# vinits5/learning3d

Measured on AMD Instinct MI355X. Metric: clouds/sec DGCNN-fwd+Chamfer B=32 N=1024; kNN HBM GB/s vs peak at 1/2/4/8 GPU, higher is better.
Workload: dtype f32 (shared-MLP GEMMs as f16x2: fp32 operands carried as an fp16 high part + an fp16 residual (unscaled between the EdgeConv kernel and conv5, 2^12-scaled elsewhere), 3 fp16 MFMA products per fp32 product, f32 accumulate, fp32-level error -- tests bound it by 2x the fp32-MFMA kernel's own error agai

## Files before the change

learning3d_amd/csrc/conv_f16.hip:

```cpp
#include <type_traits>
#include "common.h"
#include "split_bf16.h"
#include "split_f16.h"

typedef _Float16 f16x8 __attribute__((ext_vector_type(8)));

#define CF_TM 256
#define CF_TN 256
#define CF_WBYTES (6 * 4096)
#define CF_XBYTES (4 * 4096)
#define CF_STAGE (CF_WBYTES + CF_XBYTES)
#define CF_NSTAGE 3
#define CF_LDS (CF_NSTAGE * CF_STAGE)

typedef __attribute__((address_space(3))) void *cf_lds_ptr_t;
typedef const __attribute__((address_space(1))) void *cf_gbl_ptr_t;

__global__ __launch_bounds__(256) void cf_absmax_kernel(const float *__restrict__ src, size_t n, unsigned *__restrict__ out)
{
    float m = 0.f;
    const size_t gid = (size_t)blockIdx.x * 256 + threadIdx.x, gsz = (size_t)gridDim.x * 256;
    const size_t head = min(n, (size_t)((16 - ((size_t)src & 15)) & 15) / 4);
    const float4 *v = (const float4 *)(src + head);
    const size_t n4 = (n - head) / 4;
    size_t i = gid;
    for (; i + 3 * gsz < n4; i += 4 * gsz) {
        const float4 a = v[i], b = v[i + gsz], c = v[i + 2 * gsz], d = v[i + 3 * gsz];
        m = fmaxf(m, fmaxf(fmaxf(fmaxf(fabsf(a.x), fabsf(a.y)), fmaxf(fabsf(a.z), fabsf(a.w))),
                           fmaxf(fmaxf(fabsf(b.x), fabsf(b.y)), fmaxf(fabsf(b.z), fabsf(b.w)))));
        m = fmaxf(m, fmaxf(fmaxf(fmaxf(fabsf(c.x), fabsf(c.y)), fmaxf(fabsf(c.z), fabsf(c.w))),
                           fmaxf(fmaxf(fabsf(d.x), fabsf(d.y)), fmaxf(fabsf(d.z), fabsf(d.w)))));
    }
    for (; i < n4; i += gsz) {
        const float4 a = v[i];
        m = fmaxf(m, fmaxf(fmaxf(fabsf(a.x), fabsf(a.y)), fmaxf(fabsf(a.z), fabsf(a.w))));
    }
    for (size_t e = gid; e < head; e += gsz) m = fmaxf(m, fabsf(src[e]));
    for (size_t e = head + 4 * n4 + gid; e < n; e += gsz) m = fmaxf(m, fabsf(src[e]));
    for (int off = 32; off > 0; off >>= 1) m = fmaxf(m, __shfl_xor(m, off, 64));
    __shared__ float red[4];
    if ((threadIdx.x & 63) == 0) red[threadIdx.x >> 6] = m;
    __syncthreads();
    if (threadIdx.x == 0) {
        m = fmaxf(fmaxf(red[0], red[1]), fmaxf(red[2], red[3]));
        const unsigned bits = __float_as_uint(m);
        if (bits > __atomic_load_n(out, __ATOMIC_RELAXED)) atomicMax(out, bits);
    }
}

__global__ __launch_bounds__(256) void cf_absmax_rows_kernel(const float *__restrict__ src, long R, int C, long stride, unsigned *__restrict__ out)
{
    float m = 0.f;
    const long r0 = (long)blockIdx.x * 64, r1 = min(R, r0 + 64);
    for (long r = r0; r < r1; r++)
        for (int c = threadIdx.x; c < C; c += 256) m = fmaxf(m, fabsf(src[r * stride + c]));
    for (int off = 32; off > 0; off >>= 1) m = fmaxf(m, __shfl_xor(m, off, 64));
    if ((threadIdx.x & 63) == 0) atomicMax(out, __float_as_uint(m));
}

__device__ __forceinline__ int cf_clamp_exp(int s) { return s < -126 ? -126 : (s > 126 ? 126 : s); }

__device__ __forceinline__ int cf_scale_exp(float wmax)
{
    if (!(wmax > 0.f) || !(wmax < INFINITY)) return 0;
    int e;
    frexpf(wmax, &e);
    return cf_clamp_exp(3 - e);
}

__global__ __launch_bounds__(256) void cf_split_w_kernel(const float *__restrict__ src, int R, int C, const float *__restrict__ rinv,
                                                         uint4 *__restrict__ pH, uint4 *__restrict__ pHs, uint4 *__restrict__ pM)
{
    const int noct = (C + 7) / 8;
    const long id = (long)blockIdx.x * 256 + threadIdx.x;
    if (id >= (long)R * noct) return;
    const int row = (int)(id % R), o = (int)(id / R);
    const float up = 1.0f / rinv[row];
    _Float16 H[8], Hs[8], M[8];
#pragma unroll
    for (int e = 0; e < 8; e++) {
        const int k = o * 8 + e;
        const float v = (k < C ? src[(size_t)row * C + k] : 0.f) * up;
        H[e] = (_Float16)v;
        M[e] = (_Float16)(v - (float)H[e]);
        Hs[e] = (_Float16)((float)H[e] * 0x1p-12f);
    }
    pH[(size_t)o * R + row] = *(const uint4 *)H;
    pHs[(size_t)o * R + row] = *(const uint4 *)Hs;
    pM[(size_t)o * R + row] = *(const uint4 *)M;
}

__global__ __launch_bounds__(256) void cf_rowsum_kernel(const float *__restrict__ src, int R, int C, unsigned *__restrict__ out,
                                                        float *__restrict__ rinv)
{
    const int lane = threadIdx.x & 63, row = blockIdx.x * 4 + (threadIdx.x >> 6);
    float s = 0.f, mx = 0.f;
    if (row < R)
        for (int c = lane; c < C; c += 64) {
            const float a = fabsf(src[(size_t)row * C + c]);
            s += a;
            mx = fmaxf(mx, a);
        }
#pragma unroll
    for (int d = 32; d > 0; d >>= 1) {
        s += __shfl_xor(s, d, 64);
        mx = fmaxf(mx, __shfl_xor(mx, d, 64));
    }
    if (lane == 0 && row < R) rinv[row] = ldexpf(1.0f, -cf_scale_exp(mx));
    __shared__ float ws[4];
    if (lane == 0) ws[threadIdx.x >> 6] = s;
    __syncthreads();
    if (threadIdx.x == 0) atomicMax(out, __float_as_uint(fmaxf(fmaxf(ws[0], ws[1]), fmaxf(ws[2], ws[3]))));
}

__device__ __forceinline__ int cf_act_exp(float xmax)
{
    if (!(xmax > 0.f) || !(xmax < INFINITY)) return 0;
    int e;
    frexpf(xmax, &e);
    return cf_clamp_exp(12 - e);
}

__global__ __launch_bounds__(256) void cf_rowinv_act_kernel(const float *__restrict__ src, long R, int C, long stride, float *__restrict__ rinv)
{
    const int lane = threadIdx.x & 63;
    const long row = (long)blockIdx.x * 4 + (threadIdx.x >> 6);
    if (row >= R) return;
    float mx = 0.f;
    for (int c = lane; c < C; c += 64) mx = fmaxf(mx, fabsf(src[row * stride + c]));
#pragma unroll
    for (int d = 32; d > 0; d >>= 1) mx = fmaxf(mx, __shfl_xor(mx, d, 64));
    if (lane == 0) rinv[row] = ldexpf(1.0f, -cf_act_exp(mx));
}

template <bool CFIRST>
__global__ __launch_bounds__(256) void cf_split_x_kernel(const float *__restrict__ src, long R, int C, int Npts, const unsigned *__restrict__ amax,
                                                         uint4 *__restrict__ ph, uint4 *__restrict__ pm, float *__restrict__ inv,
                                                         int *__restrict__ range_flag)
{
    const int T = cf_act_exp(__uint_as_float(*amax));
    const float up = ldexpf(1.0f, T);
    if (blockIdx.x == 0 && threadIdx.x == 0) *inv = ldexpf(1.0f, -T);
    const int noct = (C + 7) / 8;
    const long id = (long)blockIdx.x * 256 + threadIdx.x;
    if (id >= R * noct) return;
    const long row = id % R;
    const int o = (int)(id / R);
    _Float16 h[8], m[8];
    float big = 0.f;
#pragma unroll
    for (int e = 0; e < 8; e++) {
        const int k = o * 8 + e;
        float v = 0.f;
        if (k < C) v = (CFIRST ? src[((size_t)(row / Npts) * C + k) * Npts + row % Npts] : src[(size_t)row * C + k]) * up;
        big = fmaxf(big, fabsf(v));
        h[e] = (_Float16)v;
        m[e] = (_Float16)((v - (float)h[e]) * 4096.0f);
    }
    ph[(size_t)o * R + row] = *(const uint4 *)h;
    pm[(size_t)o * R + row] = *(const uint4 *)m;
    if (!(big <= 60000.f) && range_flag) *(volatile int *)range_flag = 1;
}

#define CFS_ROWS 64
#define CFS_OCT 32
#define CFS_STRIDE (CFS_ROWS + 1)
__global__ __launch_bounds__(256) void cf_split_x_cl_kernel(const float *__restrict__ src, long R, int C, const unsigned *__restrict__ amax,
                                                            uint4 *__restrict__ ph, uint4 *__restrict__ pm, float *__restrict__ inv,
                                                            int *__restrict__ range_flag, long sstride = 0, float rs = 4096.0f,
                                                            const float *__restrict__ rinv = nullptr)
{
    if (sstride == 0) sstride = C;
    __shared__ uint4 lh[CFS_OCT * CFS_STRIDE], lm[CFS_OCT * CFS_STRIDE];
    const int T = cf_act_exp(__uint_as_float(*amax));
    const float up = ldexpf(1.0f, T);
    if (blockIdx.x == 0 && blockIdx.y == 0 && threadIdx.x == 0 && !rinv) *inv = ldexpf(1.0f, -T);
    const int t = threadIdx.x;
    const long row0 = (long)blockIdx.x * CFS_ROWS;
    const int o0 = blockIdx.y * CFS_OCT;
    float big = 0.f;
    {
        const int oc = t & 31, o = o0 + oc;
#pragma unroll
        for (int pass = 0; pass < CFS_ROWS / 8; pass++) {
            const int r = pass * 8 + (t >> 5);
            const long row = row0 + r;
            float v[8];
#pragma unroll
            for (int e = 0; e < 8; e++) v[e] = 0.f;
            float upr = up;
            if (row < R && o * 8 < C) {
                if (rinv) upr = 1.0f / rinv[row];
                const float *p = src + (size_t)row * sstride + o * 8;
                if (o * 8 + 8 <= C && (C & 3) == 0 && (sstride & 3) == 0 && (((size_t)src) & 15) == 0) {
                    const f32x4 a = *(const f32x4 *)p, b = *(const f32x4 *)(p + 4);
                    v[0] = a[0]; v[1] = a[1]; v[2] = a[2]; v[3] = a[3]; v[4] = b[0]; v[5] = b[1]; v[6] = b[2]; v[7] = b[3];
                } else {
#pragma unroll
                    for (int e = 0; e < 8; e++) if (o * 8 + e < C) v[e] = p[e];
                }
            }
            _Float16 h[8], m[8];
#pragma unroll
            for (int e = 0; e < 8; e++) {
                const float x = v[e] * upr;
                big = fmaxf(big, fabsf(x));
                h[e] = (_Float16)x;
                m[e] = (_Float16)((x - (float)h[e]) * rs);
            }
            lh[oc * CFS_STRIDE + r] = *(const uint4 *)h;
            lm[oc * CFS_STRIDE + r] = *(const uint4 *)m;
        }
    }
    __syncthreads();
    {
        const int r = t & 63;
        const long row = row0 + r;
        const int noct = (C + 7) / 8;
#pragma unroll
        for (int pass = 0; pass < CFS_OCT / 4; pass++) {
            const int oc = pass * 4 + (t >> 6), o = o0 + oc;
            if (row < R && o < noct) {
                ph[(size_t)o * R + row] = lh[oc * CFS_STRIDE + r];
                pm[(size_t)o * R + row] = lm[oc * CFS_STRIDE + r];
            }
        }
    }
    if (!(big <= 60000.f) && range_flag) *(volatile int *)range_flag = 1;
}

#ifdef CF_TIMELINE
__device__ long long *g_cf_timeline;
#define CFM(i) { if (threadIdx.x == 0) g_cf_timeline[(size_t)blockIdx.x * 8 + (i)] = __builtin_amdgcn_s_memrealtime(); }
#else
#define CFM(i)
#endif
template <bool NARROW, bool AMAX, bool GROUP, int NPW = 3, bool RESID = false, bool OUT2 = false, bool SHIFTN = false>
__global__ __launch_bounds__(512) void conv_f16_kernel(const uint4 *__restrict__ xh, const uint4 *__restrict__ xm,
                                                       const uint4 *__restrict__ wH, const uint4 *__restrict__ wHs,
                                                       const uint4 *__restrict__ wM, const float *__restrict__ winv,
                                                       const float *__restrict__ xinv, const float *__restrict__ scale, const float *__restrict__ shift,
                                                       int shift_bstride, int Bn, int Cin, int Cout, int N, int relu,
                                                       float *__restrict__ y, uint2 *__restrict__ oph, uint2 *__restrict__ opm,
                                                       float *__restrict__ oinv, const float *__restrict__ obs, float *__restrict__ ypool,
                                                       int pool, unsigned *__restrict__ amax_out, int amax_cdiv)
{
    constexpr int TM = NARROW ? 128 : CF_TM, TN = NARROW ? 512 : CF_TN;
    constexpr int WR = TM * 16, XR = TN * 16;
    static_assert(NPW == 3 || (NPW == 2 && !NARROW && !GROUP), "two weight planes: wide tile");
    static_assert(!RESID || (!NARROW && !AMAX && !GROUP), "residual epilogue: wide tile, fp32 output");
    static_assert(!OUT2 || (NPW == 2 && !AMAX && !RESID), "unscaled output image: the two-plane form");
    static_assert(!SHIFTN || (NPW == 2 && !AMAX && !RESID && !OUT2), "column-indexed shift: the plain two-plane form");
    constexpr int WBYTES = 2 * NPW * WR, STAGE = WBYTES + 4 * XR;
    constexpr int NPIECE = NARROW ? 6 : (NPW == 3 ? 5 : 4);
    extern __shared__ __attribute__((aligned(16))) unsigned char lds[];
    const int t = threadIdx.x, lane = t & 63, wave = t >> 6;
    const int wm = NARROW ? (wave & 1) : (wave & 3), wn = NARROW ? (wave >> 1) : (wave >> 2);
    CFM(0)
#ifdef CF_TIMELINE
    if (t == 0) { unsigned id; asm volatile("s_getreg_b32 %0, hwreg(HW_REG_HW_ID)" : "=s"(id)); g_cf_timeline[(size_t)blockIdx.x * 8 + 7] = id; }
#endif
    int pt, ct;
    {
        const int nct = Cout / TM, npt = Bn * (N / TN), L = blockIdx.x;
        if (npt % 8 == 0) {
            const int xcd = L & 7, slot = L >> 3;
            ct = slot % nct;
            pt = (slot / nct) * 8 + xcd;
        } else {
            ct = L % nct;
            pt = L / nct;
        }
    }
    const int ntn = N / TN;
    const int n0 = (pt % ntn) * TN, co0 = ct * TM, b = pt / ntn;
    const int nk = Cin / 16;
    const size_t BN = (size_t)Bn * N;

    const uint4 *src[NPIECE];
    size_t stride[NPIECE];
    int dst[NPIECE];
    constexpr int WQ = TM / 64, XQ = TN / 64, NWP = 2 * NPW * WQ, NXP = 4 * XQ;
#pragma unroll
    for (int i = 0; i < NPIECE; i++) {
        int q = wave * NPIECE + i;
        if (q >= NWP + NXP) q -= NXP;
        if (q < NWP) {
            const int reg = q / WQ, p = reg >> 1, kg = reg & 1, quarter = q % WQ;
            const uint4 *pl = p == 0 ? wH : ((NPW == 3 && p == 1) ? wHs : wM);
            src[i] = pl + (size_t)kg * Cout + co0 + quarter * 64 + lane;
            stride[i] = 2 * (size_t)Cout;
            dst[i] = reg * WR + quarter * 1024;
        } else {
            const int q2 = q - NWP, reg = q2 / XQ, p = reg >> 1, kg = reg & 1, quarter = q2 % XQ;
            const uint4 *pl = p == 0 ? xh : xm;
            src[i] = pl + (size_t)kg * BN + (size_t)b * N + n0 + quarter * 64 + lane;
            stride[i] = 2 * BN;
            dst[i] = WBYTES + reg * XR + quarter * 1024;
        }
    }
    auto issue_one = [&](int stage, int i) {
        __builtin_amdgcn_global_load_lds((cf_gbl_ptr_t)src[i], (cf_lds_ptr_t)(lds + stage * STAGE + dst[i]), 16, 0, 0);
        src[i] += stride[i];
    };
    auto issue = [&](int stage) {
#pragma unroll
        for (int i = 0; i < NPIECE; i++) issue_one(stage, i);
    };

    f32x16 acc[2][4];
#pragma unroll
    for (int a = 0; a < 2; a++)
#pragma unroll
        for (int c = 0; c < 4; c++)
#pragma unroll
            for (int r = 0; r < 16; r++) acc[a][c][r] = 0.f;

    const int kgl = lane >> 5;
    const int a_off = kgl * WR + (wm * 64 + (lane & 31)) * 16;
    const int b_off = WBYTES + kgl * XR + (wn * 128 + (lane & 31)) * 16;

    issue(0);
    if (nk > 1) issue(1);
    int stage = 0;
#ifdef CF_TIMING
    long long tq[5] = {0, 0, 0, 0, 0}, tp = __builtin_amdgcn_s_memtime();
#define CFT(n) { const long long now_ = __builtin_amdgcn_s_memtime(); tq[n] += now_ - tp; tp = now_; }
#else
#define CFT(n)
#endif
    for (int kc = 0; kc < nk; kc++) {
        CFT(4)
        if (kc + 1 >= nk) asm volatile("s_waitcnt vmcnt(0)" ::: "memory");
        else if (NARROW) asm volatile("s_waitcnt vmcnt(6)" ::: "memory");
        else if (NPW == 3) asm volatile("s_waitcnt vmcnt(5)" ::: "memory");
        else asm volatile("s_waitcnt vmcnt(4)" ::: "memory");
        CFT(0)
        __builtin_amdgcn_s_barrier();
#ifdef CF_TIMELINE
        if (kc == 0) CFM(1)
#endif
        CFT(1)
        const int nst = stage == 0 ? 2 : stage - 1;
        const bool more = kc + 2 < nk;
        CFT(2)
        const unsigned char *base = lds + stage * STAGE;
        f16x8 A[2][NPW], Bf[4][2];
#pragma unroll
        for (int p = 0; p < 2; p++)
#pragma unroll
            for (int c = 0; c < 4; c++) Bf[c][p] = *(const f16x8 *)(base + b_off + c * 512 + p * 2 * XR);
#pragma unroll
        for (int p = NPW - 1; p >= 0; p--)
#pragma unroll
            for (int a = 0; a < 2; a++) A[a][p] = *(const f16x8 *)(base + a_off + a * 512 + p * 2 * WR);
#pragma unroll
        for (int n = 0; n < 24; n++) {
            const int prod = n >> 3, a = (n >> 2) & 1, c = n & 3;
            const int pa = NPW == 3 ? (prod == 0 ? 2 : (prod == 1 ? 1 : 0)) : (prod == 0 ? 1 : 0);
            const int pb = prod == 1 ? 1 : 0;
            acc[a][c] = __builtin_amdgcn_mfma_f32_32x32x16_f16(A[a][pa], Bf[c][pb], acc[a][c], 0, 0, 0);
            constexpr int GAP = NARROW ? 4 : (NPW == 3 ? 5 : 6);
            if (n % GAP == 3) {
                __builtin_amdgcn_sched_barrier(0);
                if (more) issue_one(nst, n / GAP);
                __builtin_amdgcn_sched_barrier(0);
            }
        }
        stage = stage == 2 ? 0 : stage + 1;
        CFT(3)
    }
#ifdef CF_TIMING
    if (lane == 0) {
        long long *o = (long long *)y + ((size_t)blockIdx.x * 8 + wave) * 8;
        for (int n = 0; n < 5; n++) o[n] = tq[n];
    }
    {
        float keep = 0.f;
        for (int a = 0; a < 2; a++) for (int c = 0; c < 4; c++) for (int r = 0; r < 16; r++) keep += acc[a][c][r];
        if (keep == 12345.678f) y[0] = keep;
    }
    return;
#endif

    CFM(2)
    const float xinv0 = *xinv;
    const float *rinv = winv + 4;
    if (oph || ypool) {
        float up = 1.f;
        if (oph) {
            float bound = fmaf(obs[1] * winv[2], 4096.0f * *xinv, obs[0]) * 1.000001f;
            int e = 0;
            if (bound > 0.f && bound < 3.0e38f) (void)frexpf(bound, &e);
            const int To = cf_clamp_exp(12 - e);
            up = ldexpf(1.f, To);
            if (blockIdx.x == 0 && t == 0) *oinv = ldexpf(1.f, -To);
        }
      if constexpr (!GROUP) {
        const size_t rows = (size_t)Bn * N;
        const int half = lane >> 5, NP = N / 128;
#pragma unroll
        for (int a = 0; a < 2; a++)
#pragma unroll
            for (int gq = 0; gq < 4; gq++) {
                const int cob = co0 + wm * 64 + a * 32 + 8 * gq + 4 * half;
                float sc[4], sh[4], vmax[4];
#pragma unroll
                for (int u = 0; u < 4; u++) {
                    sc[u] = (scale ? scale[cob + u] : 1.f) * rinv[cob + u];
                    sh[u] = shift ? shift[(size_t)b * shift_bstride + cob + u] : 0.f;
                    vmax[u] = -INFINITY;
                }
#pragma unroll
                for (int c = 0; c < 4; c++) {
                    float v[4];
#pragma unroll
                    for (int u = 0; u < 4; u++) {
                        v[u] = acc[a][c][4 * gq + u] * sc[u] * xinv0 + sh[u];
                        if (relu) v[u] = l3d_act(v[u], relu);
                        vmax[u] = fmaxf(vmax[u], v[u]);
                    }
                    if (oph) {
                        uint32_t h0, h1, m0, m1;
                        if constexpr (OUT2) {
                            af_split_x_unscaled(v[0], v[1], up, h0, m0);
                            af_split_x_unscaled(v[2], v[3], up, h1, m1);
                        } else {
                            af_split_x(v[0], v[1], up, h0, m0);
                            af_split_x(v[2], v[3], up, h1, m1);
                        }
                        const size_t row = (size_t)b * N + n0 + wn * 128 + c * 32 + (lane & 31);
                        const size_t cellh = ((size_t)(cob >> 3) * rows + row) * 2 + half;
                        oph[cellh] = make_uint2(h0, h1);
                        opm[cellh] = make_uint2(m0, m1);
                    }
                }
                if (ypool) {
#pragma unroll
                    for (int u = 0; u < 4; u++) {
#pragma unroll
                        for (int d = 1; d < 32; d <<= 1) vmax[u] = fmaxf(vmax[u], __shfl_xor(vmax[u], d, 64));
                    }
                    if ((lane & 31) == 0) {
#pragma unroll
                        for (int u = 0; u < 4; u++)
                            ypool[((size_t)b * Cout + cob + u) * NP + (n0 + wn * 128) / 128] = vmax[u];
                    }
                }
            }
      } else {
        const size_t rows = (size_t)Bn * N;
        const int half = lane >> 5, NP = N / pool;
        const int span = pool < 32 ? pool : 32;
#pragma clang loop unroll(full)
        for (int a = 0; a < 2; a++)
#pragma clang loop unroll(full)
            for (int gq = 0; gq < 4; gq++) {
                const int cob = co0 + wm * 64 + a * 32 + 8 * gq + 4 * half;
                float sc[4], sh[4], pv[4][4];
#pragma unroll
                for (int u = 0; u < 4; u++) {
                    sc[u] = (scale ? scale[cob + u] : 1.f) * rinv[cob + u];
                    sh[u] = shift ? shift[(size_t)b * shift_bstride + cob + u] : 0.f;
                }
#pragma unroll
                for (int c = 0; c < 4; c++) {
                    float v[4];
#pragma unroll
                    for (int u = 0; u < 4; u++) {
                        v[u] = acc[a][c][4 * gq + u] * sc[u] * xinv0 + sh[u];
                        if (relu) v[u] = l3d_act(v[u], relu);
                        pv[c][u] = v[u];
                    }
                    if (oph) {
                        uint32_t h0, h1, m0, m1;
                        af_split_x(v[0], v[1], up, h0, m0);
                        af_split_x(v[2], v[3], up, h1, m1);
                        const size_t row = (size_t)b * N + n0 + wn * 128 + c * 32 + (lane & 31);
                        const size_t cellh = ((size_t)(cob >> 3) * rows + row) * 2 + half;
                        oph[cellh] = make_uint2(h0, h1);
                        opm[cellh] = make_uint2(m0, m1);
                    }
                }
                if (ypool) {
                    if (pool >= 64) {
#pragma unroll
                        for (int u = 0; u < 4; u++) {
                            pv[0][u] = fmaxf(pv[0][u], pv[1][u]);
                            pv[2][u] = fmaxf(pv[2][u], pv[3][u]);
                            if (pool == 128) pv[0][u] = fmaxf(pv[0][u], pv[2][u]);
                        }
                    }
                    auto finish = [&](auto c_c) {
                        constexpr int c = decltype(c_c)::value;
#pragma unroll
                        for (int u = 0; u < 4; u++) {
                            float m = pv[c][u];
#pragma unroll
                            for (int d = 1; d < 32; d <<= 1)
                                if (d < span) m = fmaxf(m, __shfl_xor(m, d, 64));
                            pv[c][u] = m;
                        }
                        if (((lane & 31) & (span - 1)) == 0) {
                            const int n = n0 + wn * 128 + c * 32 + (lane & 31);
#pragma unroll
                            for (int u = 0; u < 4; u++) ypool[((size_t)b * Cout + cob + u) * NP + n / pool] = pv[c][u];
                        }
                    };
                    finish(std::integral_constant<int, 0>{});
                    if (pool <= 64) finish(std::integral_constant<int, 2>{});
                    if (pool <= 32) { finish(std::integral_constant<int, 1>{}); finish(std::integral_constant<int, 3>{}); }
                }
            }
      }
        return;
    }
    if constexpr (GROUP) return;
    float *yb = y + (size_t)b * Cout * N;
    const float *rb = RESID ? obs + (size_t)b * Cout * N : nullptr;
    float shn[4] = {0.f, 0.f, 0.f, 0.f};
    if constexpr (SHIFTN) {
        if (shift) {
#pragma unroll
            for (int c = 0; c < 4; c++) shn[c] = shift[n0 + wn * 128 + c * 32 + (lane & 31)];
        }
    }
    float amax_nan = 0.f;
    float amax_run = 0.f;
#pragma unroll
    for (int a = 0; a < 2; a++)
#pragma unroll
        for (int r = 0; r < 16; r++) {
            const int co = co0 + wm * 64 + a * 32 + (r & 3) + 8 * (r >> 2) + 4 * (lane >> 5);
            const float sc = (scale ? scale[co] : 1.f) * rinv[co];
            const float sh = (!SHIFTN && shift) ? shift[(size_t)b * shift_bstride + co] : 0.f;
#pragma unroll
            for (int c = 0; c < 4; c++) {
                float v = acc[a][c][r] * sc * xinv0 + (SHIFTN ? shn[c] : sh);
                if (relu) v = l3d_act(v, relu);
                if constexpr (RESID) v = rb[(size_t)co * N + n0 + wn * 128 + c * 32 + (lane & 31)] + v;
                float *dst_ = &yb[(size_t)co * N + n0 + wn * 128 + c * 32 + (lane & 31)];
                if constexpr (NPW == 2 && !AMAX && !RESID && !SHIFTN) __builtin_nontemporal_store(v, dst_);
                else *dst_ = v;
                if constexpr (AMAX) {
                    asm volatile("v_max_f32_e64 %0, %0, |%1|" : "+v"(amax_run) : "v"(v));
                    asm volatile("v_fma_f32 %0, %1, 0, %0" : "+v"(amax_nan) : "v"(v));
                }
            }
        }
#ifdef CF_TIMELINE
    CFM(3)
    asm volatile("s_waitcnt vmcnt(0)" ::: "memory");
    CFM(4)
    __syncthreads();
    CFM(5)
#endif
    if constexpr (AMAX) {
        float *red = (float *)lds;
        float big = amax_run;
#pragma unroll
        for (int d = 32; d > 0; d >>= 1) big = fmaxf(big, __shfl_xor(big, d, 64));
        if (__builtin_amdgcn_ballot_w64(amax_nan != amax_nan) != 0) big = __builtin_nanf("");
        __syncthreads();
        if (lane == 0) red[wave] = big;
        __syncthreads();
        if (t == 0) {
            float m = red[0];
            for (int w = 1; w < 8; w++) m = (m != m || red[w] != red[w]) ? __builtin_nanf("") : fmaxf(m, red[w]);
            unsigned *dst = amax_out + co0 / amax_cdiv;
            if (!(m <= __uint_as_float(__atomic_load_n(dst, __ATOMIC_RELAXED)))) atomicMax(dst, __float_as_uint(m));
        }
    }
}

extern "C" size_t l3d_f16_image_bytes(int kind, long rows, int cols)
{
    return kind == 0 ? l3d_f16_plane_bytes(rows, cols) : (kind == 1 ? l3d_f16_act_bytes(rows, cols) : l3d_conv_f16_weight_bytes((int)rows, cols));
}

extern "C" int l3d_conv_f16_split_weights(const float *w, int Cout, int Cin, void *dst, l3d_stream_t stream)
{
    L3D_REQUIRE(w && dst && Cout > 0 && Cin > 0);
    hipStream_t st = (hipStream_t)stream;
    const size_t pb = l3d_f16_plane_bytes(Cout, Cin);
    unsigned char *d = (unsigned char *)dst;
    unsigned *amax = (unsigned *)(d + 3 * pb + 4);
    float *rinv = (float *)(d + 3 * pb + 16);
    if (hipMemsetAsync(d + 3 * pb, 0, 16, st) != hipSuccess) return L3D_ERR_LAUNCH;
    hipLaunchKernelGGL(cf_rowsum_kernel, dim3((unsigned)l3d_divup(Cout, 4)), dim3(256), 0, st, w, Cout, Cin, amax + 1, rinv);
    const long cells = (long)Cout * ((Cin + 7) / 8);
    hipLaunchKernelGGL(cf_split_w_kernel, dim3((unsigned)l3d_divup(cells, 256)), dim3(256), 0, st, w, Cout, Cin, (const float *)rinv,
                       (uint4 *)d, (uint4 *)(d + pb), (uint4 *)(d + 2 * pb));
    return l3d_check_launch();
}

extern "C" int l3d_split_f16_rows(const float *x, long rows, int C, int channel_first, int Npts, void *dst, int *range_flag,
                                  l3d_stream_t stream)
{
    L3D_REQUIRE(x && dst && rows > 0 && C > 0 && (!channel_first || (Npts > 0 && rows % Npts == 0)));
    hipStream_t st = (hipStream_t)stream;
    const size_t pb = l3d_f16_plane_bytes(rows, C);
    unsigned char *d = (unsigned char *)dst;
    float *inv = (float *)(d + 2 * pb);
    unsigned *amax = (unsigned *)(d + 2 * pb + 4);
    if (hipMemsetAsync(amax, 0, 4, st) != hipSuccess) return L3D_ERR_LAUNCH;
    const size_t n = (size_t)rows * C;
    const long nblk = l3d_divup((long)n, 4096);
    hipLaunchKernelGGL(cf_absmax_kernel, dim3((unsigned)(nblk > 2048 ? 2048 : nblk)), dim3(256), 0, st, x, n, amax);
    const long cells = rows * ((C + 7) / 8);
    if (channel_first)
        hipLaunchKernelGGL(cf_split_x_kernel<true>, dim3((unsigned)l3d_divup(cells, 256)), dim3(256), 0, st, x, rows, C,
                           Npts, (const unsigned *)amax, (uint4 *)d, (uint4 *)(d + pb), inv, range_flag);
    else
        hipLaunchKernelGGL(cf_split_x_cl_kernel, dim3((unsigned)l3d_divup(rows, CFS_ROWS), (unsigned)l3d_divup((C + 7) / 8, CFS_OCT)), dim3(256), 0,
                           st, x, rows, C, (const unsigned *)amax, (uint4 *)d, (uint4 *)(d + pb), inv, range_flag);
    return l3d_check_launch();
}

extern "C" int l3d_split_f16_operand(const float *x, long rows, int C, long row_stride, int kind, void *dst, int *range_flag, l3d_stream_t stream)
{
    L3D_REQUIRE(x && dst && rows > 0 && C > 0 && row_stride >= C && (kind == 0 || kind == 1));
    if ((((size_t)dst) & 15) || rows > 2147483647L) return L3D_ERR_UNSUPPORTED;
    hipStream_t st = (hipStream_t)stream;
    const size_t pb = l3d_f16_plane_bytes(rows, C);
    unsigned char *d = (unsigned char *)dst;
    uint4 *ph = (uint4 *)d, *pm = (uint4 *)(d + (kind ? 2 : 1) * pb);
    float *inv = (float *)(d + (kind ? 3 : 2) * pb);
    unsigned *amax = (unsigned *)(inv + 1);
    if (hipMemsetAsync(inv, 0, 16, st) != hipSuccess) return L3D_ERR_LAUNCH;
    float *rinv = kind ? inv + 4 : nullptr;
    if (kind) {
        hipLaunchKernelGGL(cf_rowinv_act_kernel, dim3((unsigned)l3d_divup(rows, 4L)), dim3(256), 0, st, x, rows, C, row_stride, rinv);
    } else if (row_stride == C) {
        const size_t n = (size_t)rows * C;
        const long nblk = l3d_divup((long)n, 4096);
        hipLaunchKernelGGL(cf_absmax_kernel, dim3((unsigned)(nblk > 2048 ? 2048 : nblk)), dim3(256), 0, st, x, n, amax);
    } else {
        hipLaunchKernelGGL(cf_absmax_rows_kernel, dim3((unsigned)l3d_divup(rows, 64L)), dim3(256), 0, st, x, rows, C, row_stride, amax);
    }
    hipLaunchKernelGGL(cf_split_x_cl_kernel, dim3((unsigned)l3d_divup(rows, (long)CFS_ROWS), (unsigned)l3d_divup((C + 7) / 8, CFS_OCT)), dim3(256), 0,
                       st, x, rows, C, (const unsigned *)amax, ph, pm, inv, range_flag, row_stride, 1.0f, (const float *)rinv);
    return l3d_check_launch();
}

static int cf_launch(const void *x_planes, const void *w_planes, const float *scale, const float *shift, int shift_bstride, int B,
                     int Cin, int Cout, int N, int relu, float *y, void *out_img, const float *obs, float *ypool, int pool,
                     unsigned *amax_out, int amax_cdiv, hipStream_t st, bool two_plane = false, const float *resid = nullptr,
                     bool out_unscaled = false, bool shift_n = false)
{
    const bool narrow = Cout % CF_TM != 0;
    const int tm = narrow ? 128 : CF_TM, tn = narrow ? 512 : CF_TN;
    if (Cout % tm || N % tn || Cin % 16 || B > 65535 || (((size_t)x_planes) & 15) || (((size_t)w_planes) & 15) ||
        (((size_t)out_img) & 15) || (amax_out && amax_cdiv % tm))
        return L3D_ERR_UNSUPPORTED;
    if (ypool && pool != 8 && pool != 16 && pool != 32 && pool != 64 && pool != 128) return L3D_ERR_UNSUPPORTED;
    const size_t xpb = l3d_f16_plane_bytes((long)B * N, Cin), wpb = l3d_f16_plane_bytes(Cout, Cin);
    const size_t opb = l3d_f16_plane_bytes((long)B * N, Cout);
    const unsigned char *xp = (const unsigned char *)x_planes, *wp = (const unsigned char *)w_planes;
    unsigned char *op = (unsigned char *)out_img;
    dim3 grid((unsigned)((size_t)(N / tn) * (Cout / tm) * B)), block(512);
    if (!ypool) pool = 128;
#define CF_ARGS (const uint4 *)xp, (const uint4 *)(xp + xpb), (const uint4 *)wp, (const uint4 *)(wp + wpb), (const uint4 *)(wp + 2 * wpb), \
                (const float *)(wp + 3 * wpb), (const float *)(xp + 2 * xpb), scale, shift, shift_bstride, B, Cin, Cout, N, relu, y,      \
                (uint2 *)op, op ? (uint2 *)(op + opb) : nullptr, op ? (float *)(op + 2 * opb) : nullptr, obs, ypool, pool, amax_out, amax_cdiv
    const size_t nlds = 3 * (6 * 128 * 16 + 4 * 512 * 16);
    const bool group = ypool && pool != 128;
    if (group && amax_out) return L3D_ERR_UNSUPPORTED;
    constexpr size_t lds2 = 3 * (4 * CF_TM * 16 + 4 * CF_TN * 16);
    if (out_unscaled && !(two_plane && out_img && !ypool)) return L3D_ERR_UNSUPPORTED;
    if (shift_n) {
        if (!two_plane || narrow || group || amax_out || ypool || out_img || resid || !y || shift_bstride) return L3D_ERR_UNSUPPORTED;
        hipLaunchKernelGGL((conv_f16_kernel<false, false, false, 2, false, false, true>), grid, block, lds2, st, CF_ARGS);
        return l3d_check_launch();
    }
    if (resid) {
        if (narrow || group || amax_out || ypool || out_img || !y) return L3D_ERR_UNSUPPORTED;
        obs = resid;
        if (two_plane) hipLaunchKernelGGL((conv_f16_kernel<false, false, false, 2, true>), grid, block, lds2, st, CF_ARGS);
        else hipLaunchKernelGGL((conv_f16_kernel<false, false, false, 3, true>), grid, block, CF_LDS, st, CF_ARGS);
        return l3d_check_launch();
    }
    if (two_plane && (amax_out || out_img)) {
        if (narrow || group || ypool || (amax_out && !y) || (out_img && (!out_unscaled || amax_out))) return L3D_ERR_UNSUPPORTED;
        if (amax_out) hipLaunchKernelGGL((conv_f16_kernel<false, true, false, 2>), grid, block, lds2, st, CF_ARGS);
        else hipLaunchKernelGGL((conv_f16_kernel<false, false, false, 2, false, true>), grid, block, lds2, st, CF_ARGS);
        return l3d_check_launch();
    }
    if (two_plane) {
        if (narrow || group || amax_out || ypool || out_img || !y) return L3D_ERR_UNSUPPORTED;
        hipLaunchKernelGGL((conv_f16_kernel<false, false, false, 2>), grid, block, 3 * (4 * CF_TM * 16 + 4 * CF_TN * 16), st, CF_ARGS);
        return l3d_check_launch();
    }
    if (narrow && group)         hipLaunchKernelGGL((conv_f16_kernel<true, false, true>), grid, block, nlds, st, CF_ARGS);
    else if (narrow && amax_out) hipLaunchKernelGGL((conv_f16_kernel<true, true, false>), grid, block, nlds, st, CF_ARGS);
    else if (narrow)             hipLaunchKernelGGL((conv_f16_kernel<true, false, false>), grid, block, nlds, st, CF_ARGS);
    else if (group)              hipLaunchKernelGGL((conv_f16_kernel<false, false, true>), grid, block, CF_LDS, st, CF_ARGS);
    else if (amax_out)           hipLaunchKernelGGL((conv_f16_kernel<false, true, false>), grid, block, CF_LDS, st, CF_ARGS);
    else                         hipLaunchKernelGGL((conv_f16_kernel<false, false, false>), grid, block, CF_LDS, st, CF_ARGS);
#undef CF_ARGS
    return l3d_check_launch();
}

extern "C" int l3d_pointwise_conv_f16(const void *x_planes, const void *w_planes, const float *scale, const float *shift,
                                      int shift_bstride, int B, int Cin, int Cout, int N, int relu, int flags, float *y,
                                      const float *residual, void *out_img, const float *obs, float *ypool, int pool,
                                      void *amax_out, int amax_cdiv, l3d_stream_t stream)
{
    L3D_REQUIRE(x_planes && w_planes && (y || out_img || ypool) && (!out_img || obs) && (!residual || y) && (!amax_out || (y && amax_cdiv > 0)) &&
                B > 0 && Cin > 0 && Cout > 0 && N > 0 && (flags & ~7) == 0);
    if (y && (out_img || ypool)) return L3D_ERR_UNSUPPORTED;
    return cf_launch(x_planes, w_planes, scale, shift, shift_bstride, B, Cin, Cout, N, relu, y, out_img, obs, ypool, pool,
                     (unsigned *)amax_out, amax_cdiv, (hipStream_t)stream, (flags & 1) != 0, residual, (flags & 2) != 0, (flags & 4) != 0);
}

#define CFN_MAXCIN 8
__global__ __launch_bounds__(256) void cf_first_layer_kernel(const float *__restrict__ x, int channel_last, const float *__restrict__ w,
                                                             const float *__restrict__ shift, const float *__restrict__ xmax, int Cin,
                                                             int Cout, int Npts, long R, int relu, uint4 *__restrict__ ph,
                                                             uint4 *__restrict__ pm, float *__restrict__ oinv, int *__restrict__ range_flag)
{
    __shared__ float red[4];
    const int t = threadIdx.x;
    const float xm = *xmax;
    float bnd = 0.f;
    for (int r = t; r < Cout; r += 256) {
        float s = 0.f;
        for (int c = 0; c < Cin; c++) s += fabsf(w[r * Cin + c]);
        bnd = fmaxf(bnd, fmaf(s, xm, shift ? fabsf(shift[r]) : 0.f));
    }
#pragma unroll
    for (int d = 32; d > 0; d >>= 1) bnd = fmaxf(bnd, __shfl_xor(bnd, d, 64));
    if ((t & 63) == 0) red[t >> 6] = bnd;
    __syncthreads();
    bnd = fmaxf(fmaxf(red[0], red[1]), fmaxf(red[2], red[3])) * 1.000001f;
    int e = 0;
    if (bnd > 0.f && bnd < 3.0e38f) (void)frexpf(bnd, &e);
    const int To = cf_clamp_exp(12 - e);
    const float up = ldexpf(1.f, To);
    if (blockIdx.x == 0 && blockIdx.y == 0 && t == 0) *oinv = ldexpf(1.f, -To);
    const long row = (long)blockIdx.x * 256 + t;
    const int o = blockIdx.y;
    if (row >= R) return;
    float xv[CFN_MAXCIN];
#pragma unroll
    for (int c = 0; c < CFN_MAXCIN; c++)
        xv[c] = c < Cin ? (channel_last ? x[(size_t)row * Cin + c] : x[((size_t)(row / Npts) * Cin + c) * Npts + row % Npts]) : 0.f;
    float v[8], big = 0.f;
#pragma unroll
    for (int u = 0; u < 8; u++) {
        const int co = o * 8 + u;
        float s = 0.f;
        if (co < Cout) {
#pragma unroll
            for (int c = 0; c < CFN_MAXCIN; c++)
                if (c < Cin) s = fmaf(w[co * Cin + c], xv[c], s);
            s += shift ? shift[co] : 0.f;
            if (relu) s = l3d_act(s, relu);
        }
        v[u] = s;
        big = fmaxf(big, fabsf(s * up));
    }
    uint32_t h[4], m[4];
#pragma unroll
    for (int u = 0; u < 4; u++) af_split_x(v[2 * u], v[2 * u + 1], up, h[u], m[u]);
    ph[(size_t)o * R + row] = make_uint4(h[0], h[1], h[2], h[3]);
    pm[(size_t)o * R + row] = make_uint4(m[0], m[1], m[2], m[3]);
    if (!(big <= 60000.f) && range_flag) *(volatile int *)range_flag = 1;
}

extern "C" int l3d_first_layer_f16_planes(const float *x, int channel_last, const float *w, const float *shift, const float *xmax,
                                          int B, int Cin, int Cout, int N, int relu, void *out_img, int *range_flag,
                                          l3d_stream_t stream)
{
    L3D_REQUIRE(x && w && xmax && out_img && B > 0 && Cin > 0 && Cout > 0 && N > 0);
    if (Cin > CFN_MAXCIN || (((size_t)out_img) & 15)) return L3D_ERR_UNSUPPORTED;
    const long R = (long)B * N;
    const size_t pb = l3d_f16_plane_bytes(R, Cout);
    unsigned char *d = (unsigned char *)out_img;
    dim3 grid((unsigned)l3d_divup(R, 256), (unsigned)((Cout + 7) / 8));
    hipLaunchKernelGGL(cf_first_layer_kernel, grid, dim3(256), 0, (hipStream_t)stream, x, channel_last, w, shift, xmax, Cin, Cout, N, R,
                       relu, (uint4 *)d, (uint4 *)(d + pb), (float *)(d + 2 * pb), range_flag);
    return l3d_check_launch();
}

#define GFP_ROWS 64
#define GFP_STRIDE (GFP_ROWS + 1)
template <int NO >
__global__ __launch_bounds__(256) void group_first_layer_planes_kernel(const float *__restrict__ U, const float *__restrict__ V,
                                                                       const float *__restrict__ shift, const float *__restrict__ wx,
                                                                       const float *__restrict__ xyz, const float *__restrict__ new_xyz,
                                                                       const int32_t *__restrict__ idx, int N, int S, int K, int act,
                                                                       const float *__restrict__ bound, uint4 *__restrict__ ph,
                                                                       uint4 *__restrict__ pm, float *__restrict__ oinv,
                                                                       int *__restrict__ range_flag, const float *__restrict__ maxpart,
                                                                       float wxr, float shmax)
{
    __shared__ uint4 lh[NO * GFP_STRIDE], lm[NO * GFP_STRIDE];
    __shared__ float mx4[4];
    constexpr int C1 = NO * 8, RPP = 256 / NO;
    const int t = threadIdx.x, b = blockIdx.y;
    const long SK = (long)S * K, e0 = (long)blockIdx.x * GFP_ROWS, rows = (long)gridDim.y * SK;
    int ex = 0;
    {
        float bd;
        if (maxpart) {
            float m = maxpart[t];
#pragma unroll
            for (int d = 32; d > 0; d >>= 1) m = fmaxf(m, __shfl_xor(m, d, 64));
            if ((t & 63) == 0) mx4[t >> 6] = m;
            __syncthreads();
            bd = mx4[0] + (V ? mx4[1] : shmax) + wxr * (mx4[2] + mx4[3]);
        } else {
            bd = *bound;
        }
        bd *= 1.000001f;
        if (bd > 0.f && bd < 3.0e38f) (void)frexpf(bd, &ex);
    }
    const int To = cf_clamp_exp(12 - ex);
    const float up = ldexpf(1.f, To);
    if (blockIdx.x == 0 && b == 0 && t == 0) *oinv = ldexpf(1.f, -To);
    const int oc = t % NO, r0 = t / NO;
    float w0[8], w1[8], w2[8], sh[8];
#pragma unroll
    for (int u = 0; u < 8; u++) {
        const float *w = wx + (size_t)(8 * oc + u) * 3;
        w0[u] = w[0]; w1[u] = w[1]; w2[u] = w[2];
        sh[u] = shift ? shift[8 * oc + u] : 0.f;
    }
    float big = 0.f;
#pragma unroll 2
    for (int pass = 0; pass < GFP_ROWS / RPP; pass++) {
        const int r = pass * RPP + r0;
        const long e = e0 + r;
        uint4 hc = make_uint4(0, 0, 0, 0), mc = hc;
        if (e < SK) {
            const int s_ = (int)(e / K), j = idx[(size_t)b * SK + e];
            const float *p = xyz + ((size_t)b * N + j) * 3, *q = new_xyz + ((size_t)b * S + s_) * 3;
            const float dx = p[0] - q[0], dy = p[1] - q[1], dz = p[2] - q[2];
            const f32x4 *up4 = (const f32x4 *)(U + ((size_t)b * N + j) * C1 + 8 * oc);
            f32x4 ua = up4[0], ub = up4[1];
            if (V) {
                const f32x4 *vp4 = (const f32x4 *)(V + ((size_t)b * S + s_) * C1 + 8 * oc);
                ua += vp4[0]; ub += vp4[1];
            }
            float v[8];
#pragma unroll
            for (int u = 0; u < 8; u++) {
                float x = (u < 4 ? ua[u] : ub[u - 4]) + sh[u];
                x = fmaf(w2[u], dz, fmaf(w1[u], dy, fmaf(w0[u], dx, x)));
                if (act) x = l3d_act(x, act);
                v[u] = x;
                big = fmaxf(big, fabsf(x * up));
            }
            af_split_x(v[0], v[1], up, hc.x, mc.x);
            af_split_x(v[2], v[3], up, hc.y, mc.y);
            af_split_x(v[4], v[5], up, hc.z, mc.z);
            af_split_x(v[6], v[7], up, hc.w, mc.w);
        }
        lh[oc * GFP_STRIDE + r] = hc;
        lm[oc * GFP_STRIDE + r] = mc;
    }
    __syncthreads();
    {
        const int r = t & 63;
        const long e = e0 + r;
        if (e < SK) {
            const size_t row = (size_t)b * SK + e;
#pragma unroll
            for (int pass = 0; pass < NO / 4; pass++) {
                const int o = pass * 4 + (t >> 6);
                ph[(size_t)o * rows + row] = lh[o * GFP_STRIDE + r];
                pm[(size_t)o * rows + row] = lm[o * GFP_STRIDE + r];
            }
        }
    }
    if (!(big <= 60000.f) && range_flag) *(volatile int *)range_flag = 1;
}

static int gfp_launch(const float *U, const float *V, const float *shift, const float *wx, const float *xyz, const float *new_xyz,
                      const int32_t *idx, int B, int N, int S, int K, int C1, int relu, const float *bound, const float *maxpart,
                      float wxr, float shmax, void *out_img, int *range_flag, hipStream_t st)
{
    if (B > 65535 || (C1 != 64 && C1 != 128 && C1 != 256) || (((size_t)U | (size_t)V | (size_t)out_img) & 15)) return L3D_ERR_UNSUPPORTED;
    const long R = (long)B * S * K;
    const size_t pb = l3d_f16_plane_bytes(R, C1);
    unsigned char *d = (unsigned char *)out_img;
    dim3 grid((unsigned)l3d_divup((long)S * K, GFP_ROWS), B), block(256);
#define GFP_ARGS U, V, shift, wx, xyz, new_xyz, idx, N, S, K, relu, bound, (uint4 *)d, (uint4 *)(d + pb), (float *)(d + 2 * pb), range_flag, \
                 maxpart, wxr, shmax
    if (C1 == 64)       hipLaunchKernelGGL(group_first_layer_planes_kernel<8>, grid, block, 0, st, GFP_ARGS);
    else if (C1 == 128) hipLaunchKernelGGL(group_first_layer_planes_kernel<16>, grid, block, 0, st, GFP_ARGS);
    else                hipLaunchKernelGGL(group_first_layer_planes_kernel<32>, grid, block, 0, st, GFP_ARGS);
#undef GFP_ARGS
    return l3d_check_launch();
}

__global__ __launch_bounds__(256) void absmax4_partials_kernel(const float *__restrict__ p0, size_t n0, const float *__restrict__ p1,
                                                               size_t n1, const float *__restrict__ p2, size_t n2,
                                                               const float *__restrict__ p3, size_t n3, float *__restrict__ out)
{
    __shared__ float red[4];
    const int j = blockIdx.y;
    const float *p = j == 0 ? p0 : (j == 1 ? p1 : (j == 2 ? p2 : p3));
    const size_t n = j == 0 ? n0 : (j == 1 ? n1 : (j == 2 ? n2 : n3));
    float m = 0.f;
    if (p) {
        const size_t n4 = (((size_t)p & 15) == 0) ? n >> 2 : 0;
        for (size_t i = (size_t)blockIdx.x * 256 + threadIdx.x; i < n4; i += (size_t)gridDim.x * 256) {
            const float4 v = ((const float4 *)p)[i];
            m = fmaxf(fmaxf(m, fmaxf(fabsf(v.x), fabsf(v.y))), fmaxf(fabsf(v.z), fabsf(v.w)));
        }
        for (size_t i = (n4 << 2) + (size_t)blockIdx.x * 256 + threadIdx.x; i < n; i += (size_t)gridDim.x * 256) m = fmaxf(m, fabsf(p[i]));
    }
#pragma unroll
    for (int d = 32; d > 0; d >>= 1) m = fmaxf(m, __shfl_xor(m, d, 64));
    if ((threadIdx.x & 63) == 0) red[threadIdx.x >> 6] = m;
    __syncthreads();
    if (threadIdx.x == 0) out[j * 64 + blockIdx.x] = fmaxf(fmaxf(red[0], red[1]), fmaxf(red[2], red[3]));
}

extern "C" int l3d_absmax4_partials(const float *p0, size_t n0, const float *p1, size_t n1, const float *p2, size_t n2,
                                    const float *p3, size_t n3, float *out, l3d_stream_t stream)
{
    L3D_REQUIRE(out);
    hipLaunchKernelGGL(absmax4_partials_kernel, dim3(64, 4), dim3(256), 0, (hipStream_t)stream, p0, n0, p1, n1, p2, n2, p3, n3, out);
    return l3d_check_launch();
}

extern "C" int l3d_group_first_layer_planes_auto(const float *U, const float *V, const float *shift, const float *wx, const float *xyz,
                                                 const float *new_xyz, const int32_t *idx, int B, int N, int S, int K, int C1, int relu,
                                                 const float *maxpart, float wxr, float shmax, void *out_img, int *range_flag,
                                                 l3d_stream_t stream)
{
    L3D_REQUIRE(U && wx && xyz && new_xyz && idx && maxpart && out_img && B > 0 && N > 0 && S > 0 && K > 0 && C1 > 0);
    return gfp_launch(U, V, shift, wx, xyz, new_xyz, idx, B, N, S, K, C1, relu, nullptr, maxpart, wxr, shmax, out_img, range_flag,
                      (hipStream_t)stream);
}
```

Before: 116,900.

## Add tail-split two-plane f16 conv kernel with 4-stage pipeline and fused epilogue

Adds a dedicated kernel for the plain two-plane f16x2 pointwise conv path. It runs a four-stage global_load_lds pipeline over all but the last three K chunks, then consumes those three resident chunks interleaved with the epilogue so the final MFMAs overlap the scale/shift/ReLU and nontemporal stores. The goal is to hide the pipeline drain and epilogue latency at the end of the K loop. It also adds a route query function and header. The cost is extra LDS (four stages) and possibly lower occupancy, and the change only applies when Cin/16 is at least 5.

```diff
diff --git a/include/ext/l3d_conv_f16_route.h b/include/ext/l3d_conv_f16_route.h
--- /dev/null
+++ b/include/ext/l3d_conv_f16_route.h
@@ -0,0 +1,17 @@
+#ifndef L3D_CONV_F16_ROUTE_H
+#define L3D_CONV_F16_ROUTE_H
+#include "../l3d_hip.h"
+#ifdef __cplusplus
+extern "C" {
+#endif
+
+#define L3D_CONV_F16_ROUTE_LOOP 0
+#define L3D_CONV_F16_ROUTE_TAIL 1
+#define L3D_CONV_F16_TAIL_CHUNKS 3
+
+int l3d_conv_f16_route(int Cin, int Cout, int N, int flags);
+
+#ifdef __cplusplus
+}
+#endif
+#endif
diff --git a/learning3d_amd/csrc/conv_f16.hip b/learning3d_amd/csrc/conv_f16.hip
--- a/learning3d_amd/csrc/conv_f16.hip
+++ b/learning3d_amd/csrc/conv_f16.hip
@@ -2,6 +2,7 @@
 #include "common.h"
 #include "split_bf16.h"
 #include "split_f16.h"
+#include "../../include/ext/l3d_conv_f16_route.h"
 
 typedef _Float16 f16x8 __attribute__((ext_vector_type(8)));
 
@@ -12,6 +13,7 @@
 #define CF_STAGE (CF_WBYTES + CF_XBYTES)
 #define CF_NSTAGE 3
 #define CF_LDS (CF_NSTAGE * CF_STAGE)
+#define CF_TAIL L3D_CONV_F16_TAIL_CHUNKS
 
 typedef __attribute__((address_space(3))) void *cf_lds_ptr_t;
 typedef const __attribute__((address_space(1))) void *cf_gbl_ptr_t;
@@ -573,6 +575,170 @@
     }
 }
 
+#define CFT_STAGE (4 * CF_TM * 16 + 4 * CF_TN * 16)
+#define CFT_LDS (4 * CFT_STAGE + 2 * CF_TM * (int)sizeof(float))
+__global__ __launch_bounds__(512) void conv_f16_tail_kernel(const uint4 *__restrict__ xh, const uint4 *__restrict__ xm,
+                                                            const uint4 *__restrict__ wH, const uint4 *__restrict__ wM,
+                                                            const float *__restrict__ winv, const float *__restrict__ xinv,
+                                                            const float *__restrict__ scale, const float *__restrict__ shift,
+                                                            int shift_bstride, int Bn, int Cin, int Cout, int N, int relu, float *__restrict__ y)
+{
+    constexpr int WR = CF_TM * 16, XR = CF_TN * 16, WBYTES = 4 * WR, STAGE = CFT_STAGE, NPIECE = 4, T = CF_TAIL;
+    static_assert(CF_TM == 256 && CF_TN == 256 && T == 3, "32 pieces of 64 rows per chunk, four per wave; stage arithmetic mod 4");
+    extern __shared__ __attribute__((aligned(16))) unsigned char lds[];
+    const int t = threadIdx.x, lane = t & 63, wave = t >> 6;
+    const int wm = wave & 3, wn = wave >> 2;
+    CFM(0)
+#ifdef CF_TIMELINE
+    if (t == 0) { unsigned id; asm volatile("s_getreg_b32 %0, hwreg(HW_REG_HW_ID)" : "=s"(id)); g_cf_timeline[(size_t)blockIdx.x * 8 + 7] = id; }
+#endif
+    int pt, ct;
+    {
+        const int nct = Cout / CF_TM, npt = Bn * (N / CF_TN), L = blockIdx.x;
+        if (npt % 8 == 0) {
+            const int xcd = L & 7, slot = L >> 3;
+            ct = slot % nct;
+            pt = (slot / nct) * 8 + xcd;
+        } else {
+            ct = L % nct;
+            pt = L / nct;
+        }
+    }
+    const int ntn = N / CF_TN;
+    const int n0 = (pt % ntn) * CF_TN, co0 = ct * CF_TM, b = pt / ntn;
+    const int nk = Cin / 16;
+    const size_t BN = (size_t)Bn * N;
+
+    const uint4 *src[NPIECE];
+    size_t stride[NPIECE];
+    int dst[NPIECE];
+#pragma unroll
+    for (int i = 0; i < NPIECE; i++) {
+        const int q = wave * NPIECE + i, reg = (q & 15) >> 2, p = reg >> 1, kg = reg & 1, quarter = q & 3;
+        if (q < 16) {
+            src[i] = (p == 0 ? wH : wM) + (size_t)kg * Cout + co0 + quarter * 64 + lane;
+            stride[i] = 2 * (size_t)Cout;
+            dst[i] = reg * WR + quarter * 1024;
+        } else {
+            src[i] = (p == 0 ? xh : xm) + (size_t)kg * BN + (size_t)b * N + n0 + quarter * 64 + lane;
+            stride[i] = 2 * BN;
+            dst[i] = WBYTES + reg * XR + quarter * 1024;
+        }
+    }
+    auto issue_one = [&](int stage, int i) {
+        __builtin_amdgcn_global_load_lds((cf_gbl_ptr_t)src[i], (cf_lds_ptr_t)(lds + stage * STAGE + dst[i]), 16, 0, 0);
+        src[i] += stride[i];
+    };
+
+    f32x16 acc[2][4];
+#pragma unroll
+    for (int a = 0; a < 2; a++)
+#pragma unroll
+        for (int c = 0; c < 4; c++)
+#pragma unroll
+            for (int r = 0; r < 16; r++) acc[a][c][r] = 0.f;
+
+    const int kgl = lane >> 5;
+    const int a_off = kgl * WR + (wm * 64 + (lane & 31)) * 16;
+    const int b_off = WBYTES + kgl * XR + (wn * 128 + (lane & 31)) * 16;
+
+#pragma unroll
+    for (int i = 0; i < NPIECE; i++) issue_one(0, i);
+#pragma unroll
+    for (int i = 0; i < NPIECE; i++) issue_one(1, i);
+    float *csc = (float *)(lds + 4 * STAGE), *csh = csc + CF_TM;
+    if (t < CF_TM) {
+        csc[t] = (scale ? scale[co0 + t] : 1.f) * winv[4 + co0 + t];
+        csh[t] = shift ? shift[(size_t)b * shift_bstride + co0 + t] : 0.f;
+    }
+    const float xinv0 = *xinv;
+    for (int kc = 0; kc < nk - T; kc++) {
+        const bool last = kc == nk - T - 1, prev = kc == nk - T - 2;
+        if (last) asm volatile("s_waitcnt vmcnt(8)" ::: "memory");
+        else asm volatile("s_waitcnt vmcnt(4)" ::: "memory");
+        __builtin_amdgcn_s_barrier();
+#ifdef CF_TIMELINE
+        if (kc == 0) CFM(1)
+#endif
+        const int ust = last ? ((kc + 3) & 3) : ((kc + 2) & 3), est = (kc + 3) & 3;
+        const unsigned char *base = lds + (kc & 3) * STAGE;
+        f16x8 A[2][2], Bf[4][2];
+#pragma unroll
+        for (int p = 0; p < 2; p++)
+#pragma unroll
+            for (int c = 0; c < 4; c++) Bf[c][p] = *(const f16x8 *)(base + b_off + c * 512 + p * 2 * XR);
+#pragma unroll
+        for (int p = 1; p >= 0; p--)
+#pragma unroll
+            for (int a = 0; a < 2; a++) A[a][p] = *(const f16x8 *)(base + a_off + a * 512 + p * 2 * WR);
+#pragma unroll
+        for (int n = 0; n < 24; n++) {
+            const int prod = n >> 3, a = (n >> 2) & 1, c = n & 3;
+            acc[a][c] = __builtin_amdgcn_mfma_f32_32x32x16_f16(A[a][prod == 0 ? 1 : 0], Bf[c][prod == 1 ? 1 : 0], acc[a][c], 0, 0, 0);
+            if (n % 6 == 3) {
+                __builtin_amdgcn_sched_barrier(0);
+                issue_one(ust, n / 6);
+                __builtin_amdgcn_sched_barrier(0);
+            }
+            if (n % 6 == 5) {
+                __builtin_amdgcn_sched_barrier(0);
+                if (prev) issue_one(est, n / 6);
+                __builtin_amdgcn_sched_barrier(0);
+            }
+        }
+    }
+    asm volatile("s_waitcnt vmcnt(0)" ::: "memory");
+    __builtin_amdgcn_s_barrier();
+    CFM(2)
+    const int wmu = __builtin_amdgcn_readfirstlane(wm), wnu = __builtin_amdgcn_readfirstlane(wn);
+    float *yu = y + ((size_t)b * Cout + co0 + wmu * 64) * N + n0 + wnu * 128;
+    const unsigned voff = (unsigned)(4 * kgl) * (unsigned)N + (unsigned)(lane & 31);
+    const unsigned char *cb[T];
+#pragma unroll
+    for (int j = 0; j < T; j++) cb[j] = lds + ((nk - T + j) & 3) * STAGE;
+    const float *lsc = csc + wm * 64 + 4 * kgl, *lsh = csh + wm * 64 + 4 * kgl;
+#pragma unroll
+    for (int a = 0; a < 2; a++) {
+        f16x8 A[T][2];
+#pragma unroll
+        for (int j = 0; j < T; j++)
+#pragma unroll
+            for (int p = 0; p < 2; p++) A[j][p] = *(const f16x8 *)(cb[j] + a_off + a * 512 + p * 2 * WR);
+#pragma unroll
+        for (int c = 0; c < 4; c++) {
+            f16x8 Bf[T][2];
+#pragma unroll
+            for (int j = 0; j < T; j++)
+#pragma unroll
+                for (int p = 0; p < 2; p++) Bf[j][p] = *(const f16x8 *)(cb[j] + b_off + c * 512 + p * 2 * XR);
+#pragma unroll
+            for (int j = 0; j < T; j++) {
+                acc[a][c] = __builtin_amdgcn_mfma_f32_32x32x16_f16(A[j][1], Bf[j][0], acc[a][c], 0, 0, 0);
+                acc[a][c] = __builtin_amdgcn_mfma_f32_32x32x16_f16(A[j][0], Bf[j][1], acc[a][c], 0, 0, 0);
+                acc[a][c] = __builtin_amdgcn_mfma_f32_32x32x16_f16(A[j][0], Bf[j][0], acc[a][c], 0, 0, 0);
+            }
+#pragma unroll
+            for (int g = 0; g < 4; g++) {
+                const f32x4 sc4 = *(const f32x4 *)(lsc + a * 32 + 8 * g), sh4 = *(const f32x4 *)(lsh + a * 32 + 8 * g);
+#pragma unroll
+                for (int u = 0; u < 4; u++) {
+                    float v = acc[a][c][4 * g + u] * sc4[u] * xinv0 + sh4[u];
+                    if (relu) v = l3d_act(v, relu);
+                    __builtin_nontemporal_store(v, yu + (size_t)(a * 32 + u + 8 * g) * N + c * 32 + voff);
+                }
+            }
+            __builtin_amdgcn_sched_barrier(0);
+        }
+    }
+#ifdef CF_TIMELINE
+    CFM(3)
+    asm volatile("s_waitcnt vmcnt(0)" ::: "memory");
+    CFM(4)
+    __syncthreads();
+    CFM(5)
+#endif
+}
+
 extern "C" size_t l3d_f16_image_bytes(int kind, long rows, int cols)
 {
     return kind == 0 ? l3d_f16_plane_bytes(rows, cols) : (kind == 1 ? l3d_f16_act_bytes(rows, cols) : l3d_conv_f16_weight_bytes((int)rows, cols));
@@ -642,6 +808,8 @@
                        st, x, rows, C, (const unsigned *)amax, ph, pm, inv, range_flag, row_stride, 1.0f, (const float *)rinv);
     return l3d_check_launch();
 }
+
+static bool cf_tail_route(int Cin) { return Cin / 16 >= CF_TAIL + 2; }
 
 static int cf_launch(const void *x_planes, const void *w_planes, const float *scale, const float *shift, int shift_bstride, int B,
                      int Cin, int Cout, int N, int relu, float *y, void *out_img, const float *obs, float *ypool, int pool,
@@ -688,6 +856,12 @@
     }
     if (two_plane) {
         if (narrow || group || amax_out || ypool || out_img || !y) return L3D_ERR_UNSUPPORTED;
+        if (cf_tail_route(Cin)) {
+            hipLaunchKernelGGL(conv_f16_tail_kernel, grid, block, CFT_LDS, st, (const uint4 *)xp, (const uint4 *)(xp + xpb), (const uint4 *)wp,
+                               (const uint4 *)(wp + 2 * wpb), (const float *)(wp + 3 * wpb), (const float *)(xp + 2 * xpb), scale, shift,
+                               shift_bstride, B, Cin, Cout, N, relu, y);
+            return l3d_check_launch();
+        }
         hipLaunchKernelGGL((conv_f16_kernel<false, false, false, 2>), grid, block, 3 * (4 * CF_TM * 16 + 4 * CF_TN * 16), st, CF_ARGS);
         return l3d_check_launch();
     }
@@ -711,6 +885,15 @@
     if (y && (out_img || ypool)) return L3D_ERR_UNSUPPORTED;
     return cf_launch(x_planes, w_planes, scale, shift, shift_bstride, B, Cin, Cout, N, relu, y, out_img, obs, ypool, pool,
                      (unsigned *)amax_out, amax_cdiv, (hipStream_t)stream, (flags & 1) != 0, residual, (flags & 2) != 0, (flags & 4) != 0);
+}
+
+extern "C" int l3d_conv_f16_route(int Cin, int Cout, int N, int flags)
+{
+    L3D_REQUIRE(Cin > 0 && Cout > 0 && N > 0 && (flags & ~7) == 0);
+    const bool narrow = Cout % CF_TM != 0;
+    if (Cout % (narrow ? 128 : CF_TM) || N % (narrow ? 512 : CF_TN) || Cin % 16 || (flags & 2) || ((flags & 4) && !(flags & 1)) || ((flags & 1) && narrow))
+        return L3D_ERR_UNSUPPORTED;
+    return (flags == 1 && cf_tail_route(Cin)) ? L3D_CONV_F16_ROUTE_TAIL : L3D_CONV_F16_ROUTE_LOOP;
 }
 
 #define CFN_MAXCIN 8
```

Result: faster. 119,200, median of 6 (+2.0%).
